# tsinghua-fib-lab/PIML

Hardware: AMD Instinct MI355X
Metric: agent-pair force evals/sec + simulated steps/sec, 4096-agent GC scene (higher is better)
Workload: dtype f32

## Files before the change

include/piml_hip_tuning.h:

```cpp
#ifndef PIML_HIP_TUNING_H
#define PIML_HIP_TUNING_H

#include "piml_hip.h"

#ifdef __cplusplus
extern "C" {
#endif

int piml_timer_create(void** event);
int piml_timer_record(void* event, void* stream);
int piml_timer_elapsed_ms(void* start, void* stop, float* ms);
int piml_timer_destroy(void* event);

int piml_trace_begin(void);
int piml_trace_mark(const char* name, void* stream);
int piml_trace_end(char* names, int names_cap, float* us, int us_cap);

int piml_probe_arith(const float* rx, const float* ry, const float* hx, const float* hy,
                     float* dist, float* cosv, int n, void* stream);

long long piml_encoder_split_tiles(long long tiles);
long long piml_encoder_split_tiles_train(long long tiles);
int piml_encoder_products(int split_bf16);
int piml_rowdecoder_products(int split_bf16);
int piml_encoder_dw2(int layer_split);
int piml_encoder_fused_bwd(int on);
int piml_encoder_sums_bwd(int form);
int piml_encoder_sums_dec_slots(int on);
int piml_encoder_compact_rows(int on);
int piml_relfeat_pack_form(int form);
int piml_relfeat_pack_plan(int form, int waves, int obstacle_workgroups, int nbr, int has_head, int has_fold, int skip_f32,
                           int* pack_blocks, int* share);
int piml_relfeat_pack_tail_blocks(int b, int nb, int total, int* out, int cap);
int piml_relfeat_plan(int C, int N, int M, int focal_count, int topk_ped, int topk_obs, int part, int has_pack, int* waves,
                      int* resident, int* split, int* agent_tiles, int* obstacle_tiles);
int piml_pinnsf_streams_init(void);

#ifdef __cplusplus
}
#endif
#endif
```

piml_amd/_lib.py:

```python
import ctypes
import os

import torch

_HERE = os.path.dirname(os.path.abspath(__file__))
LIB_PATH = os.environ.get('PIML_LIB') or os.path.join(_HERE, 'libpiml_hip.so')
ABI_VERSION = 35
COMPACT_MAX_AGENTS = 16384
COMPACT_SLOTS = 256

_lib = None

_i, _f, _p, _z = ctypes.c_int, ctypes.c_float, ctypes.c_void_p, ctypes.c_size_t
_ll = ctypes.c_longlong
_d = ctypes.c_double


class EncoderBranch(ctypes.Structure):
    _fields_ = [('x', _p), ('rows', _ll), ('in_dim', _i), ('k', _i),
                ('w1', _p), ('b1', _p), ('w2', _p), ('b2', _p), ('w3', _p), ('b3', _p),
                ('scale', _f), ('h1', _p), ('h2', _p), ('msgs', _p), ('g_pooled', _p), ('g_msgs', _p),
                ('g2', _p), ('g1', _p), ('g_x', _p), ('partials', _p), ('grads', _p), ('packed', _p), ('relu_mask', _p),
                ('keep_bits', _p), ('drop_state', _p), ('drop_p', _f), ('sum_a', _p), ('sum_b', _p),
                ('nbr_idx', _p), ('plan', _p)]
# ... 201 lines not shown
    'piml_colsum_blocks': [_z, _i],
    'piml_act_bwd_colsum': [_p, _p, _z, _i, _p, _p, _p, _p],
    'piml_sum_leading': [_p, _i, _z, _p, _p],
    'piml_act_bwd_colsum_stage1': [_p, _p, _z, _i, _p, _p, _p, _p],
    'piml_layer_reduce': [_p, _i, _z, _p, _p, _i, _i, _p, _p],
    'piml_scale_ksum_fwd': [_p, _p, _z, _i, _i, _f, _p, _p, _p, _p],
    'piml_ksum_blocks': [_z, _i],
    'piml_scale_ksum_bwd': [_p, _p, _z, _i, _i, _f, _p, _p, _p, _p],
    'piml_dropout_keep_bits': [_p, _ll, _i, _f, _i, _p, _p],
    'piml_timer_create': [ctypes.POINTER(_p)],
    'piml_timer_record': [_p, _p],
    'piml_timer_elapsed_ms': [_p, _p, ctypes.POINTER(_f)],
    'piml_timer_destroy': [_p],
    'piml_trace_begin': [],
    'piml_trace_mark': [ctypes.c_char_p, _p],
    'piml_trace_end': [ctypes.c_char_p, _i, ctypes.POINTER(_f), _i],
    'piml_probe_arith': [_p, _p, _p, _p, _p, _p, _i, _p],
    'piml_encoder_partial_floats': [],
    'piml_encoder_pack_floats': [],
    'piml_encoder_split_tiles': [_ll],
    'piml_encoder_split_tiles_train': [_ll],
    'piml_multi_copy': [ctypes.POINTER(_p), ctypes.POINTER(_p), ctypes.POINTER(_z), _i, _p],
    'piml_rollout_prologue': [_p] * 8 + [_i] * 4 + [_p] * 11 + [_p],
    'piml_rollout_losses_blocks': [_i, _i],
    'piml_rollout_losses': [_p, _p, _ll, _p, _p, _p, _p, _p, _i, _i, _i, _f, _p, _p, _p, _p, _p, _p, _p],
    'piml_rollout_losses_bwd': [_p, _p, _p, _p, _p, _p, _ll, _p, _p],
    'piml_rollout_losses_frames': [_p, _p, _ll, _p, _p, ctypes.POINTER(_p), _i, _p, _i, _i, _i, _f, _f, _f, _p, _p, _p, _p, _p, _p, _p],
    'piml_rollout_losses_frames_bwd': [_p, _p, _p, _p, _f, _f, _p, _p, _p, _ll, _p, _p],
    'piml_collision_pred_loss_blocks': [_ll, _i],
    'piml_collision_pred_loss': [ctypes.POINTER(_p), ctypes.POINTER(_p), _i, _ll, _i, _i, _p, _i, _i, _f, _p, _p, _p, _p, _p],
    'piml_collision_pred_loss_bwd': [_p, _p, _ll, _p, _p],
    'piml_adam_tickets': [],
    'piml_adam_step': [ctypes.POINTER(_p)] * 5 + [ctypes.POINTER(_ll), _i, ctypes.c_double, ctypes.c_double, ctypes.c_double, ctypes.c_double, ctypes.c_double, _p, _p],
    'piml_pointwise_losses_blocks': [_ll, _ll, _i],
    'piml_pointwise_losses': [_p, _p, _ll, _ll, _p, _ll, _f, _p, _i, _p, _p, _p, _p, _p],
    'piml_p2p_alloc': [_z, ctypes.POINTER(_p)],
    'piml_p2p_free': [_p],
    'piml_p2p_export': [_p, _p],
    'piml_p2p_open': [_p, ctypes.POINTER(_p)],
    'piml_p2p_close': [_p],
    'piml_p2p_copy': [_p, _p, _z, _p],
    'piml_allgather_state_p2p': [_p, _z, _i, _i, ctypes.POINTER(_p), ctypes.POINTER(_p), ctypes.c_uint, ctypes.c_uint, _p, _p],
    'piml_encoder_products': [_i],
    'piml_relfeat_pack_form': [_i],
    'piml_relfeat_pack_plan': [_i, _i, _i, _i, _i, _i, _i, ctypes.POINTER(_i), ctypes.POINTER(_i)],
    'piml_relfeat_pack_tail_blocks': [_i, _i, _i, ctypes.POINTER(_i), _i],
    'piml_relfeat_plan': [_i] * 8 + [ctypes.POINTER(_i)] * 5,
    'piml_rowdecoder_products': [_i],
    'piml_encoder_dw2': [_i],
    'piml_encoder_fused_bwd': [_i],
    'piml_encoder_sums_bwd': [_i],
    'piml_encoder_sums_dec_slots': [_i],
    'piml_encoder_compact_rows': [_i],
    'piml_encoder_pack': [ctypes.POINTER(EncoderBranch), _i, _p],
    'piml_encoder_workgroups': [ctypes.POINTER(EncoderBranch), _i, ctypes.POINTER(_i)],
    'piml_encoder_fwd': [ctypes.POINTER(EncoderBranch), _i, _p],
    'piml_encoder_fwd_packed': [ctypes.POINTER(EncoderBranch), _i, _p],
    'piml_encoder_bwd': [ctypes.POINTER(EncoderBranch), _i, _p],
    'piml_encoder_bwd_acc': [ctypes.POINTER(EncoderBranch), _i, _i, _p],
    'piml_encoder_ksum': [_p, _ll, _i, _p, _p],
    'piml_decoder_pack_floats': [],
    'piml_decoder_partial_floats': [],
    'piml_decoder_workgroups': [_ll],
    'piml_decoder_fwd': [ctypes.POINTER(DecoderBranch), _i, _p, _f, _p, _p],
    'piml_decoder_bwd': [ctypes.POINTER(DecoderBranch), _i, _p, _p, _f, _p, _p],
    'piml_rowdecoder_slots': [_ll],
    'piml_rowdecoder_fwd': [ctypes.POINTER(DecoderBranch), _i, _p],
    'piml_rowdecoder_fwd_packed': [ctypes.POINTER(DecoderBranch), _i, _p],
    'piml_rowdecoder_bwd': [ctypes.POINTER(DecoderBranch), _i, _p],
    'piml_rowdecoder_bwd_acc': [ctypes.POINTER(DecoderBranch), _i, _i, _p],
    'piml_collision_head_pack_floats': [],
    'piml_collision_head_fwd': [_p, _ll, _p, _p, _p, _p, _p, _p, _p],
    'piml_head64_partial_floats': [],
    'piml_head64_slots': [_ll],
    'piml_head64_fwd': [ctypes.POINTER(Head64), _p],
    'piml_head64_bwd': [ctypes.POINTER(Head64), _p],
    'piml_head64_bwd_acc': [ctypes.POINTER(Head64), _i, _p],
    'piml_corrector_partial_floats': [_i],
    'piml_corrector_slots': [_i, _ll, _i],
    'piml_corrector_fwd': [ctypes.POINTER(Corrector), _p],
    'piml_corrector_bwd': [ctypes.POINTER(Corrector), _i, _p],
    'piml_pinnsf_pool_h2_ok': [ctypes.POINTER(EncoderBranch), _i],
    'piml_pinnsf_pool_train_ok': [ctypes.POINTER(EncoderBranch), _i],
    'piml_pinnsf_pool_msgs_ok': [ctypes.POINTER(EncoderBranch), _i],
    'piml_pinnsf_streams_init': [],
    'piml_pinnsf_pack_flush': [],
    'piml_pinnsf_slot_sums_flush': [],
    'piml_pinnsf_pack': [ctypes.POINTER(EncoderBranch), ctypes.POINTER(DecoderBranch), _i, ctypes.POINTER(CollisionHead),
                         _i, _p],
    'piml_pinnsf_fwd': [ctypes.POINTER(EncoderBranch), ctypes.POINTER(DecoderBranch), _i, ctypes.POINTER(CollisionHead),
                        _p, _f, _p, _i, _p],
    'piml_pinnsf_bwd': [ctypes.POINTER(EncoderBranch), ctypes.POINTER(DecoderBranch), _i, _p, _p, _f, _p, _i, _p],
    'piml_comm_available': [],
    'piml_comm_unique_id': [_p],
    'piml_comm_init': [ctypes.POINTER(_p), _i, _i, _p],
    'piml_comm_destroy': [_p],
    'piml_allgather_state': [_p, _p, _z, _p, _p],
    'piml_reducescatter_grad': [_p, _p, _p, _z, _p],
    'piml_allreduce_sum': [_p, _p, _z, _p],
    'piml_relfeat_fwd_self': [_p, _p, _p, _p, _i, _p, _p, _p, _i, _i, _i, _i, _i, _i, _i, _f, _f, _f, _f, _p, _p, _p, _p, _p, _p, _p],
    'piml_relfeat_bwd_self': [_p, _p, _p, _p, _p, _p, _i, _p, _i, _i, _i, _i, _i, _i, _p, _p, _p, _p],
    'piml_relfeat_fwd_tick': [_p, _p, _p, _p, _i, _p, _p, _i, _i, _i, _i, _i, _i, _i, _f, _f, _f, _f,
                              _p, _p, _p, _i, _p, _p, _p, _p],
    'piml_relfeat_self_fwd': [_p, _p, _p, _p, _i, _i, _i, _i, _i, _i, _f, _f, _f, _f, _p, _p, _p, _p, _p, _p, _p],
    'piml_relfeat_self_fwd_part': [_i, _p, _p, _p, _p, _i, _i, _i, _i, _i, _i, _f, _f, _f, _f, _p, _p, _p, _p, _p, _p, _p],
    'piml_relfeat_self_bwd': [_p, _p, _p, _p, _p, _p, _p, _i, _i, _i, _i, _i, _p, _p, _p, _p],
# ... 167 lines not shown
```

piml_amd/csrc/encoder_x3.hip:

```cpp
#include <cstdlib>

#include "common.hpp"
#include "encoder.hpp"
#include "philox.hpp"
#include "x3.hpp"

namespace piml {

struct Pieces {
    u32x4 hi[8], mid[8], lo[8];
};

__device__ __forceinline__ void split_tile(const f32x16 (&in)[4], Pieces& P) {
#pragma unroll
    for (int kb = 0; kb < 8; ++kb) {
        const f32x16& a = in[kb >> 1];
        const int r = 8 * (kb & 1);
        unsigned hi[4], mid[4], lo[4];
#pragma unroll
        for (int d = 0; d < 4; ++d) split3(a[r + 2 * d], a[r + 2 * d + 1], hi[d], mid[d], lo[d]);
        P.hi[kb] = (u32x4){hi[0], hi[1], hi[2], hi[3]};
        P.mid[kb] = (u32x4){mid[0], mid[1], mid[2], mid[3]};
        P.lo[kb] = (u32x4){lo[0], lo[1], lo[2], lo[3]};
    }
// ... 89 lines not shown
}
__device__ __forceinline__ void pool_block_k(const f32x16& ab, int blk, int k, long long tile, long long agents, int lane,
                                             float* __restrict__ part_a, float* __restrict__ part_b) {
    if (k == 6) {
        switch ((int)(tile % 3)) {
            case 0: pool_block<6, 0>(ab, blk, tile, agents, lane, part_a, part_b); break;
            case 1: pool_block<6, 1>(ab, blk, tile, agents, lane, part_a, part_b); break;
            default: pool_block<6, 2>(ab, blk, tile, agents, lane, part_a, part_b); break;
        }
    } else if (k == 10) {
        switch ((int)(tile % 5)) {
            case 0: pool_block<10, 0>(ab, blk, tile, agents, lane, part_a, part_b); break;
            case 1: pool_block<10, 1>(ab, blk, tile, agents, lane, part_a, part_b); break;
            case 2: pool_block<10, 2>(ab, blk, tile, agents, lane, part_a, part_b); break;
            case 3: pool_block<10, 3>(ab, blk, tile, agents, lane, part_a, part_b); break;
            default: pool_block<10, 4>(ab, blk, tile, agents, lane, part_a, part_b); break;
        }
    } else {
        pool_block<2, 0>(ab, blk, tile, agents, lane, part_a, part_b);
    }
}
__device__ __forceinline__ void store_rows_block(const f32x16& ab, int blk, float* __restrict__ out, long long tile, long long R, int lane) {
    const int j = lane & 31, h = lane >> 5;
    float* __restrict__ base = out + (tile * 32 + 4 * h) * EH + 32 * blk + j;
    const long long left = R - tile * 32 - 4 * h;
    if (R - tile * 32 >= 32) {
#pragma unroll
        for (int r = 0; r < 16; ++r) base[((r & 3) + 8 * (r >> 2)) * EH] = ab[r];
    } else {
#pragma unroll
        for (int r = 0; r < 16; ++r)
            if ((r & 3) + 8 * (r >> 2) < left) base[((r & 3) + 8 * (r >> 2)) * EH] = ab[r];
    }
}

__device__ __forceinline__ void pool_rows_k(const f32x16 (&a)[4], int k, long long tile, long long agents, int lane, float* __restrict__ part_a,
                                            float* __restrict__ part_b) {
    if (k == 6) {
        switch ((int)(tile % 3)) {
            case 0: pool_rows<6, 0>(a, tile, agents, lane, part_a, part_b); break;
            case 1: pool_rows<6, 1>(a, tile, agents, lane, part_a, part_b); break;
            default: pool_rows<6, 2>(a, tile, agents, lane, part_a, part_b); break;
        }
    } else if (k == 10) {
        switch ((int)(tile % 5)) {
            case 0: pool_rows<10, 0>(a, tile, agents, lane, part_a, part_b); break;
            case 1: pool_rows<10, 1>(a, tile, agents, lane, part_a, part_b); break;
            case 2: pool_rows<10, 2>(a, tile, agents, lane, part_a, part_b); break;
            case 3: pool_rows<10, 3>(a, tile, agents, lane, part_a, part_b); break;
            default: pool_rows<10, 4>(a, tile, agents, lane, part_a, part_b); break;
        }
    } else {
        pool_rows<2, 0>(a, tile, agents, lane, part_a, part_b);
    }
}

template <int DROP, bool EXCH = false>
__global__ __launch_bounds__(ENC_THREADS) void enc_fwd_x3_kernel(EncArgs A) {
    extern __shared__ __align__(16) float lds[];
    const int tid = threadIdx.x, lane = tid & 63, wave = uniform((int)(threadIdx.x >> 6));
    const int b = (A.nbr > 1 && (int)blockIdx.x >= A.wg_split) ? 1 : 0;
    const piml_encoder_branch J = b ? A.br[1] : A.br[0];
    const int wg0 = b ? A.wg_split : 0;
    const int nwg = b ? (int)gridDim.x - A.wg_split : (A.nbr > 1 ? A.wg_split : (int)gridDim.x);
    const long long R = J.rows;
    const int IN = J.in_dim;
    const long long ntiles = (R + 31) >> 5;
    const long long first = (long long)wave * nwg + ((int)blockIdx.x - wg0);
    const long long stride = (long long)nwg * ENC_WAVES;
    if (A.zero)
        for (int e = blockIdx.x * ENC_THREADS + tid; e < A.zero_n; e += gridDim.x * ENC_THREADS) A.zero[e] = 0.f;
    unsigned long long gseed = 0, goff = 0;
    if (DROP == 2) { gseed = A.gen_state[0]; goff = A.gen_state[1]; }
    if ((long long)((int)blockIdx.x - wg0) >= ntiles) {
        if (DROP == 2 && tid == 0) dropout_advance(A.gen_state, goff, gridDim.x);
        return;
    }

    const float* x3 = J.packed + PACK_F32;
    float xb[4];
    ENC_STAMP(0, false);
    load_x(xb, J.x, first, ntiles, R, IN, lane);
    stage_linear<X3_IMG>(lds, x3, tid);
    stage_linear<1024 + 384>(lds + X3_FWD_F32, J.packed + 32768, tid);
    __syncthreads();
    u32x4 w3r[W3_ROUNDS];
    {
        const u32x4* src = reinterpret_cast<const u32x4*>(x3 + X3_IMG);
#pragma unroll
        for (int r = 0; r < W3_ROUNDS; ++r) {
            const int e = r * ENC_THREADS + tid;
            w3r[r] = src[e < W3_N4 ? e : 0];
        }
    }
    bool w3_pending = true;
    ENC_STAMP(1, false);
    if (EXCH && DROP) {
        land_w3(w3r, lds, tid);
        w3_pending = false;
    }
    ENC_STAMP(2, false);

    for (long long tile = first; tile < ntiles; tile += stride) {
        int lane_t = lane;
        asm volatile("" : "+v"(lane_t));
        const u32x4* W2hm = reinterpret_cast<const u32x4*>(lds) + lane_t;
// ... 174 lines not shown
    ENC_STAMP(7, false);
    ENC_STAMP(8, true);
    if (w3_pending) land_w3(w3r, lds, tid);
    if (DROP == 2 && tid == 0) dropout_advance(A.gen_state, goff, gridDim.x);
}

__device__ __forceinline__ float add_halves(float x) {
    const unsigned u = __float_as_uint(x);
    const auto r = __builtin_amdgcn_permlane32_swap(u, u, false, false);
    return __uint_as_float(r[0]) + __uint_as_float(r[1]);
}

template <int K, int PH>
__device__ __forceinline__ void pool_rows(const f32x16 (&a)[4], long long tile, long long agents, int lane, float* __restrict__ part_a,
                                          float* __restrict__ part_b) {
    constexpr int o = (PH * 32) % K;
    constexpr int S = (o + 31) / K + 1;
    const int i = lane & 31;
    const bool h = lane >= 32;
    const long long a0 = (tile * 32) / K;
    float tot[4][S];
#pragma unroll
    for (int blk = 0; blk < 4; ++blk) {
        float sum[S];
#pragma unroll
        for (int s = 0; s < S; ++s) sum[s] = 0.f;
#pragma unroll
        for (int r = 0; r < 16; ++r) {
            const int m0 = (r & 3) + 8 * (r >> 2), s0 = (o + m0) / K, s1 = (o + m0 + 4) / K;
            if (s0 == s1) sum[s0] += a[blk][r];
            else {
                sum[s0] += h ? 0.f : a[blk][r];
                sum[s1] += h ? a[blk][r] : 0.f;
            }
        }
#pragma unroll
        for (int s = 0; s < S; ++s) tot[blk][s] = add_halves(sum[s]);
    }
    float* __restrict__ pa = part_a + a0 * EH + i;
    float* __restrict__ pb = part_b + a0 * EH + i;
    const int left = (int)(agents - a0 < S ? agents - a0 : S);
    if (!h) {
#pragma unroll
        for (int s = 0; s < S; ++s) {
            if (s < left) {
                float* dst = (s == 0 && o != 0) ? pb : pa;
#pragma unroll
                for (int blk = 0; blk < 4; ++blk) dst[s * EH + 32 * blk] = tot[blk][s];
            }
        }
    }
}

__global__ __launch_bounds__(ENC_THREADS) void enc_fwd_pool_x3_kernel(EncArgs A) {
    extern __shared__ __align__(16) float lds[];
    const int tid = threadIdx.x, lane = tid & 63, wave = uniform((int)(threadIdx.x >> 6));
    const int b = (A.nbr > 1 && (int)blockIdx.x >= A.wg_split) ? 1 : 0;
    const piml_encoder_branch J = b ? A.br[1] : A.br[0];
    const int wg0 = b ? A.wg_split : 0;
    const int nwg = b ? (int)gridDim.x - A.wg_split : (A.nbr > 1 ? A.wg_split : (int)gridDim.x);
    const long long R = J.rows;
    const int IN = J.in_dim;
    const long long ntiles = (R + 31) >> 5;
    const long long first = (long long)wave * nwg + ((int)blockIdx.x - wg0);
    const long long stride = (long long)nwg * ENC_WAVES;
    if (A.zero)
        for (int e = blockIdx.x * ENC_THREADS + tid; e < A.zero_n; e += gridDim.x * ENC_THREADS) A.zero[e] = 0.f;
    if ((long long)((int)blockIdx.x - wg0) >= ntiles) return;
    const float* x3 = J.packed + PACK_F32;
    float xb[4];
    load_x(xb, J.x, first, ntiles, R, IN, lane);
    stage_linear<X3_IMG>(lds, x3, tid);
    stage_linear<1024 + 384>(lds + X3_FWD_F32, J.packed + 32768, tid);
    __syncthreads();
    const int k = J.k;
    const long long agents = R / k;
    for (long long tile = first; tile < ntiles; tile += stride) {
        int lane_t = lane;
        asm volatile("" : "+v"(lane_t));
        const u32x4* W2hm = reinterpret_cast<const u32x4*>(lds) + lane_t;
        const u32x4* W2lo = W2hm + X3_HM / 4;
        const float* W1f = lds + X3_FWD_F32;
        const float* bias = W1f + 1024;
        const int h = lane_t >> 5;
        f32x16 a[4];
        Pieces P;
#pragma unroll
        for (int blk = 0; blk < 4; ++blk) {
#pragma unroll
            for (int q = 0; q < 4; ++q) {
                const float4 bq = *reinterpret_cast<const float4*>(bias + feat0(blk, q, h));
                a[blk][4 * q + 0] = bq.x; a[blk][4 * q + 1] = bq.y; a[blk][4 * q + 2] = bq.z; a[blk][4 * q + 3] = bq.w;
            }
#pragma unroll
            for (int s = 0; s < 4; ++s) a[blk] = mfma32(W1f[(blk * 4 + s) * 64 + lane_t], xb[s], a[blk]);
            const float pre0 = a[blk][0];
#pragma unroll
            for (int r = 0; r < 16; ++r) a[blk][r] = relu1(a[blk][r]);
            if (blk == 0) a[0][0] = __builtin_fmaf(pre0, 0.f, a[0][0]);
        }
        split_tile(a, P);
        load_x(xb, J.x, tile + stride, ntiles, R, IN, lane);
#pragma unroll
        for (int blk = 0; blk < 4; ++blk) {
            f32x16 acc, sm;
            const float bv = bias[128 + 32 * blk + (lane_t & 31)];
#pragma unroll
            for (int r = 0; r < 16; ++r) { sm[r] = 0.f; acc[r] = bv; }
#pragma unroll
            for (int kb = 0; kb < 8; ++kb) {
                const int fb = blk * 8 + kb;
                kblock_x3_t(acc, sm, W2hm[(fb * 2) * 64], W2hm[(fb * 2 + 1) * 64], W2lo[fb * 64], P.hi[kb], P.mid[kb], P.lo[kb]);
            }
#pragma unroll
            for (int r = 0; r < 16; ++r) {
                const float pre = acc[r] + sm[r];
                a[blk][r] = blk == 0 ? __builtin_fmaf(pre, 0.f, relu1(pre)) : relu1(pre);
            }
        }
        pool_rows_k(a, k, tile, agents, lane_t, J.msgs, J.h2);
    }
}


template <bool ROWS>
__device__ __forceinline__ void store_h2_rows(const f32x16 (&a)[4], float* __restrict__ h2, long long tile, long long R, int lane) {
    if (!ROWS) return;
    const int j = lane & 31, h = lane >> 5;
    float* __restrict__ base = h2 + (tile * 32 + 4 * h) * EH + j;
    const long long left = R - tile * 32 - 4 * h;
    if (R - tile * 32 >= 32) {
#pragma unroll
        for (int blk = 0; blk < 4; ++blk)
#pragma unroll
            for (int r = 0; r < 16; ++r) base[((r & 3) + 8 * (r >> 2)) * EH + 32 * blk] = a[blk][r];
    } else {
#pragma unroll
        for (int blk = 0; blk < 4; ++blk)
#pragma unroll
            for (int r = 0; r < 16; ++r)
                if ((r & 3) + 8 * (r >> 2) < left) base[((r & 3) + 8 * (r >> 2)) * EH + 32 * blk] = a[blk][r];
    }
}

constexpr int CP_LDS_CNT = X3_IMG;
constexpr int CP_LDS_LIST = X3_IMG + 1024;
constexpr int CP_ROUNDS0 = 8;
static_assert((CP_LDS_LIST - X3_IMG) * 4 + PIML_COMPACT_MAX_AGENTS * 2 <= (X3_FWD_F32 - X3_IMG) * 4, "the lists fit W3's region");
static_assert(PIML_COMPACT_MAX_AGENTS <= 65536 && PIML_COMPACT_MAX_AGENTS <= 32 * ENC_THREADS, "u16 entries, a 32-bit flag word per thread");

__device__ __forceinline__ bool cp_straddles(int agent, int k) { return ((agent * k) >> 5) != ((agent * k + k - 1) >> 5); }

__device__ __forceinline__ unsigned cp_split_cost(int w0, int tiles0, int tiles1, int nemp) {
    const int w1 = PIML_COMPACT_SLOTS - w0;
    const unsigned c0 = (unsigned)((tiles0 + w0 - 1) / w0) * 6000u;
    const unsigned c1 = (unsigned)((tiles1 + w1 - 1) / w1) * 6000u + (nemp > 0 ? 2500u + 40u * (unsigned)((nemp + w1 - 1) / w1) : 0u);
    return min(c0 > c1 ? c0 : c1, (1u << 23) - 1u);
}

template <int K>
__device__ __forceinline__ void pool_rows_c(const f32x16 (&a)[4], int tile, int nne, const unsigned short* list, int lane,
                                            float* __restrict__ sum_a, float* __restrict__ sum_b) {
    constexpr int S = 32 / K;
    const int i = lane & 31;
    const bool h = lane >= 32;
    float tot[4][S];
#pragma unroll
    for (int blk = 0; blk < 4; ++blk) {
        float sum[S];
#pragma unroll
        for (int s = 0; s < S; ++s) sum[s] = 0.f;
#pragma unroll
        for (int r = 0; r < 16; ++r) {
            const int m0 = (r & 3) + 8 * (r >> 2), s0 = m0 / K, s1 = (m0 + 4) / K;
            if (s0 == s1) {
                if (s0 < S) sum[s0] += a[blk][r];
            } else {
                if (s0 < S) sum[s0] += h ? 0.f : a[blk][r];
                if (s1 < S) sum[s1] += h ? a[blk][r] : 0.f;
            }
        }
#pragma unroll
        for (int s = 0; s < S; ++s) tot[blk][s] = add_halves(sum[s]);
    }
    const int left = nne - S * tile;
    if (!h) {
#pragma unroll
        for (int s = 0; s < S; ++s) {
            if (s < left) {
                const int ag = list[S * tile + s];
                float* __restrict__ dst = sum_a + (size_t)ag * EH + i;
#pragma unroll
                for (int blk = 0; blk < 4; ++blk) dst[32 * blk] = tot[blk][s];
                if (cp_straddles(ag, K)) {
                    float* __restrict__ zb = sum_b + (size_t)ag * EH + i;
#pragma unroll
                    for (int blk = 0; blk < 4; ++blk) zb[32 * blk] = 0.f;
                }
            }
        }
    }
}

template <bool CP>
__device__ __forceinline__ void enc_fwd_sum_body(const EncArgs& A) {
    extern __shared__ __align__(16) float lds[];
    const int tid = threadIdx.x, lane = tid & 63, wave = uniform((int)(threadIdx.x >> 6));
    const int b = (A.nbr > 1 && (int)blockIdx.x >= A.wg_split) ? 1 : 0;
    const piml_encoder_branch J = b ? A.br[1] : A.br[0];
    const int wg0 = b ? A.wg_split : 0;
    const int nwg = b ? (int)gridDim.x - A.wg_split : (A.nbr > 1 ? A.wg_split : (int)gridDim.x);
    const long long R = J.rows;
    const int IN = J.in_dim;
    const bool cp = CP && b == 1;
    long long ntiles = (R + 31) >> 5;
    const long long first = (long long)wave * nwg + ((int)blockIdx.x - wg0);
    const long long stride = (long long)nwg * ENC_WAVES;
    if (A.zero)
        for (int e = blockIdx.x * ENC_THREADS + tid; e < A.zero_n; e += gridDim.x * ENC_THREADS) A.zero[e] = 0.f;
    if (!cp && (long long)((int)blockIdx.x - wg0) >= ntiles) return;
    const float* x3 = J.packed + PACK_F32;
    float xb[4];
    ENC_STAMP(0, false);
    const int k = J.k;
    const int agents = CP ? (int)(R / k) : 0;
    int iv[CP_ROUNDS0];
    if (cp) {
#pragma unroll
        for (int i = 0; i < CP_ROUNDS0; ++i) {
            const int a = i * ENC_THREADS + tid;
            iv[i] = a < agents ? J.nbr_idx[(size_t)a * k] : -1;
        }
    } else {
        load_x(xb, J.x, first, ntiles, R, IN, lane);
    }
    stage_linear<X3_IMG>(lds, x3, tid);
    stage_linear<1024 + 384>(lds + X3_FWD_F32, J.packed + 32768, tid);
    ENC_STAMP(1, true);
    int nne = 0, nemp = 0, S = 1, slot_n = 0, kn = 0;
    bool rowlive = false;
    const unsigned short* list = reinterpret_cast<const unsigned short*>(lds + CP_LDS_LIST);
    if (cp) {
        int* cnt = reinterpret_cast<int*>(lds + CP_LDS_CNT);
        unsigned short* lw = reinterpret_cast<unsigned short*>(lds + CP_LDS_LIST);
        const int rounds = (agents + ENC_THREADS - 1) / ENC_THREADS;
        unsigned flags = 0;
#pragma unroll
        for (int i = 0; i < CP_ROUNDS0; ++i) flags |= (iv[i] >= 0 ? 1u : 0u) << i;
        for (int i = CP_ROUNDS0; i < rounds; ++i) {
            const int a = i * ENC_THREADS + tid;
            const int v = a < agents ? J.nbr_idx[(size_t)a * k] : -1;
            flags |= (v >= 0 ? 1u : 0u) << i;
        }
        for (int i = 0; i < rounds; ++i) {
            const unsigned long long bal = __ballot((flags >> i) & 1u);
            if (lane == 0) cnt[i * ENC_WAVES + wave] = __popcll(bal);
        }
// ... 39 lines not shown
            for (int c = tid; c < nne; c += ENC_THREADS) J.plan[CP_LISTS + c] = list[c];
            for (int e = tid; e < nemp; e += ENC_THREADS) J.plan[CP_LISTS + apad + e] = list[agents - 1 - e];
            __syncthreads();
            if (tid == 0) {
                const int w0 = cnt[257] & 255;
                J.plan[0] = nne; J.plan[1] = nemp; J.plan[2] = (int)ntiles; J.plan[3] = w0; J.plan[4] = PIML_COMPACT_SLOTS - w0;
            }
        }
    } else {
        __syncthreads();
    }
    ENC_STAMP(2, false);
    auto load_xc = [&](long long tile) {
        const int idx = S * (int)tile + slot_n;
        const bool ok = tile < ntiles && rowlive && idx < nne;
        const long long row = ok ? (long long)list[idx] * k + kn : 0;
#pragma unroll
        for (int s = 0; s < 4; ++s) {
            const int c = 2 * s + (lane >> 5);
            xb[s] = (ok && c < IN) ? J.x[row * IN + c] : 0.f;
        }
    };
    if (cp) load_xc(first);
    const long long agents_d = R / k;
    for (long long tile = first; tile < ntiles; tile += stride) {
        int lane_t = lane;
        asm volatile("" : "+v"(lane_t));
        const u32x4* W2hm = reinterpret_cast<const u32x4*>(lds) + lane_t;
        const u32x4* W2lo = W2hm + X3_HM / 4;
        const float* W1f = lds + X3_FWD_F32;
        const float* bias = W1f + 1024;
        const int h = lane_t >> 5;
        f32x16 a[4];
        Pieces P;
#pragma unroll
        for (int blk = 0; blk < 4; ++blk) {
#pragma unroll
            for (int q = 0; q < 4; ++q) {
                const float4 bq = *reinterpret_cast<const float4*>(bias + feat0(blk, q, h));
                a[blk][4 * q + 0] = bq.x; a[blk][4 * q + 1] = bq.y; a[blk][4 * q + 2] = bq.z; a[blk][4 * q + 3] = bq.w;
            }
#pragma unroll
            for (int s = 0; s < 4; ++s) a[blk] = mfma32(W1f[(blk * 4 + s) * 64 + lane_t], xb[s], a[blk]);
#pragma unroll
            for (int r = 0; r < 16; ++r) a[blk][r] = relu1(a[blk][r]);
        }
        uint2* mrow = reinterpret_cast<uint2*>(J.relu_mask) + (tile * 2) * 64 + lane_t;
        mrow[0] = make_uint2(sign_bits(a[0], a[1]), sign_bits(a[2], a[3]));
        ENC_STAMP(3, false);
        split_tile(a, P);
        ENC_STAMP(4, false);
        if (cp) load_xc(tile + stride);
        else load_x(xb, J.x, tile + stride, ntiles, R, IN, lane);
#pragma unroll
        for (int blk = 0; blk < 4; ++blk) {
            f32x16 acc, sm;
            const float bv = bias[128 + 32 * blk + (lane_t & 31)];
#pragma unroll
            for (int r = 0; r < 16; ++r) { sm[r] = 0.f; acc[r] = bv; }
#pragma unroll
            for (int kb = 0; kb < 8; ++kb) {
                const int fb = blk * 8 + kb;
                kblock_x3_t(acc, sm, W2hm[(fb * 2) * 64], W2hm[(fb * 2 + 1) * 64], W2lo[fb * 64], P.hi[kb], P.mid[kb], P.lo[kb]);
            }
#pragma unroll
            for (int r = 0; r < 16; ++r) a[blk][r] = relu1(acc[r] + sm[r]);
        }
        ENC_STAMP(5, false);
        mrow[64] = make_uint2(sign_bits(a[0], a[1]), sign_bits(a[2], a[3]));
        if (J.h2) store_h2_rows<true>(a, J.h2, tile, R, lane_t);
        ENC_STAMP(6, false);
        if (cp) {
            if (k == 10) pool_rows_c<10>(a, (int)tile, nne, list, lane_t, J.sum_a, J.sum_b);
            else if (k == 6) pool_rows_c<6>(a, (int)tile, nne, list, lane_t, J.sum_a, J.sum_b);
            else pool_rows_c<2>(a, (int)tile, nne, list, lane_t, J.sum_a, J.sum_b);
        } else {
            pool_rows_k(a, k, tile, agents_d, lane_t, J.sum_a, J.sum_b);
        }
        ENC_STAMP(7, false);
    }
    if (cp && nemp > 0) {
        const int nwav = nwg * ENC_WAVES, idle = nwav - (int)ntiles;
        const int q = idle > 0 ? (int)first - (int)ntiles : (int)first, share = idle > 0 ? idle : nwav;
        if (q >= 0) {
            const float2 hc = reinterpret_cast<const float2*>(J.packed + PACK_ZROW + EH)[lane];
            const float2 v = make_float2((float)k * hc.x, (float)k * hc.y);
            for (int e = q; e < nemp; e += share) {
                const int ag = list[agents - 1 - e];
                reinterpret_cast<float2*>(J.sum_a + (size_t)ag * EH)[lane] = v;
                if (cp_straddles(ag, k)) reinterpret_cast<float2*>(J.sum_b + (size_t)ag * EH)[lane] = make_float2(0.f, 0.f);
            }
        }
    }
    ENC_STAMP(8, true);
}
__global__ __launch_bounds__(ENC_THREADS) void enc_fwd_sum_x3_kernel(EncArgs A) { enc_fwd_sum_body<false>(A); }
__global__ __launch_bounds__(ENC_THREADS) void enc_fwd_sum_x3_cp_kernel(EncArgs A) { enc_fwd_sum_body<true>(A); }

constexpr int X3_SPLIT_LDS_BYTES = 2 * 2 * 4 * 3 * 2 * 64 * 16;

template <int DROP>
__global__ __launch_bounds__(512) void enc_fwd_split_x3_kernel(EncArgs A, int pairs0) {
    extern __shared__ __align__(16) float lds[];
    u32x4* exch = reinterpret_cast<u32x4*>(lds);
    const int tid = threadIdx.x, lane = tid & 63, wave = __builtin_amdgcn_readfirstlane(tid >> 6);
    const int b = (int)blockIdx.x >= pairs0 ? 1 : 0;
    const piml_encoder_branch J = b ? A.br[1] : A.br[0];
    const int t = wave >> 2, blk = wave & 3;
    const long long R = J.rows;
    const int IN = J.in_dim;
    const long long tile = ((long long)blockIdx.x - (b ? pairs0 : 0)) * 2 + t;
    const int j = lane & 31, h = lane >> 5;
    const long long row = tile * 32 + j;
    const bool valid = row < R;
    if (A.zero)
        for (int e = blockIdx.x * 512 + tid; e < A.zero_n; e += gridDim.x * 512) A.zero[e] = 0.f;
    const unsigned long long goff = DROP == 2 ? A.gen_state[1] : 0ull;
    const u32x4* W2hm = reinterpret_cast<const u32x4*>(J.packed + PACK_F32) + lane;
    const u32x4* W2lo = W2hm + X3_HM / 4;
    const u32x4* W3hm = reinterpret_cast<const u32x4*>(J.packed + PACK_F32 + X3_IMG) + lane;
    const u32x4* W3lo = W3hm + X3_HM / 4;
    const float* W1g = J.packed + 32768;
    const float* bias = J.packed + 32768 + 1024;
    u32x4 wf[8][3];
#pragma unroll
    for (int kb = 0; kb < 8; ++kb) {
        const int fb = blk * 8 + kb;
        wf[kb][0] = W2hm[(fb * 2) * 64]; wf[kb][1] = W2hm[(fb * 2 + 1) * 64]; wf[kb][2] = W2lo[fb * 64];
    }
    float xb[4], w1[4];
#pragma unroll
    for (int s = 0; s < 4; ++s) {
        const int c = 2 * s + h;
        xb[s] = (valid && c < IN) ? J.x[(valid ? row : 0) * IN + c] : 0.f;
        w1[s] = W1g[(blk * 4 + s) * 64 + lane];
    }
    float4 bq[4], bqn[4];
#pragma unroll
    for (int q = 0; q < 4; ++q) bq[q] = *reinterpret_cast<const float4*>(bias + feat0(blk, q, h));
    f32x16 acc, sm;
    auto init = [&]() {
#pragma unroll
        for (int q = 0; q < 4; ++q) { acc[4 * q] = bq[q].x; acc[4 * q + 1] = bq[q].y; acc[4 * q + 2] = bq[q].z; acc[4 * q + 3] = bq[q].w; }
#pragma unroll
        for (int r = 0; r < 16; ++r) sm[r] = 0.f;
    };
    auto store = [&](float* dst, float sc) {
        if (dst && valid) {
            float* o = dst + row * EH;
#pragma unroll
// ... 422 lines not shown
        __syncthreads();
    }
    if (blk == 0 && J.g_x) {
        float gx[8];
#pragma unroll
        for (int c = 0; c < 8; ++c) gx[c] = 0.f;
#pragma unroll
        for (int bp = 0; bp < 4; ++bp)
#pragma unroll
            for (int q = 0; q < 4; ++q) {
                __builtin_amdgcn_sched_barrier(0);
#pragma unroll
                for (int u = 0; u < 4; ++u) {
                    const int f = feat0(bp, q, h) + u;
                    const float4 wa = W1r[2 * f], wb = W1r[2 * f + 1];
                    const float v = g1x[((t * 4 + bp) * 16 + 4 * q + u) * 64 + lane];
                    gx[0] = __fmaf_rn(wa.x, v, gx[0]); gx[1] = __fmaf_rn(wa.y, v, gx[1]);
                    gx[2] = __fmaf_rn(wa.z, v, gx[2]); gx[3] = __fmaf_rn(wa.w, v, gx[3]);
                    gx[4] = __fmaf_rn(wb.x, v, gx[4]); gx[5] = __fmaf_rn(wb.y, v, gx[5]);
                    gx[6] = __fmaf_rn(wb.z, v, gx[6]); gx[7] = __fmaf_rn(wb.w, v, gx[7]);
                }
            }
#pragma unroll
        for (int c = 0; c < 8; ++c) gx[c] += __shfl_xor(gx[c], 32, 64);
        if (valid) {
            float* o = J.g_x + row * IN + 4 * h;
            const int left = IN - 4 * h;
            const float s0 = h ? gx[4] : gx[0], s1 = h ? gx[5] : gx[1], s2 = h ? gx[6] : gx[2], s3 = h ? gx[7] : gx[3];
            if (left > 0) o[0] = s0;
            if (left > 1) o[1] = s1;
            if (left > 2) o[2] = s2;
            if (left > 3) o[3] = s3;
        }
    }
}


int enc_x3_set_attributes() {
    auto set = [](const void* f, int bytes) { return (int)hipFuncSetAttribute(f, hipFuncAttributeMaxDynamicSharedMemorySize, bytes); };
    if (int e = set(reinterpret_cast<const void*>(enc_bwd_dx_split_x3_kernel<false>), X3_DXS_LDS_BYTES)) return e;
    if (int e = set(reinterpret_cast<const void*>(enc_bwd_dx_split_x3_kernel<true>), X3_DXS_LDS_BYTES)) return e;
    if (int e = set(reinterpret_cast<const void*>(enc_fwd_split_x3_kernel<0>), X3_SPLIT_LDS_BYTES)) return e;
    if (int e = set(reinterpret_cast<const void*>(enc_fwd_split_x3_kernel<1>), X3_SPLIT_LDS_BYTES)) return e;
    if (int e = set(reinterpret_cast<const void*>(enc_fwd_split_x3_kernel<2>), X3_SPLIT_LDS_BYTES)) return e;
    const void* dx[4] = {reinterpret_cast<const void*>(enc_bwd_dx_x3_kernel<false, false>),
                         reinterpret_cast<const void*>(enc_bwd_dx_x3_kernel<true, false>),
                         reinterpret_cast<const void*>(enc_bwd_dx_x3_kernel<false, true>),
                         reinterpret_cast<const void*>(enc_bwd_dx_x3_kernel<true, true>)};
    for (const void* f : dx)
        if (int e = set(f, X3_DX_LDS_BYTES)) return e;
    if (int e = set(reinterpret_cast<const void*>(enc_fwd_pool_x3_kernel), X3_FWD_LDS_BYTES)) return e;
    if (int e = set(reinterpret_cast<const void*>(enc_fwd_sum_x3_kernel), X3_FWD_LDS_BYTES)) return e;
    if (int e = set(reinterpret_cast<const void*>(enc_fwd_sum_x3_cp_kernel), X3_FWD_LDS_BYTES)) return e;
    if (int e = set(reinterpret_cast<const void*>(enc_fwd_x3_kernel<2, true>), X3_FWD_LDS_BYTES)) return e;
    if (int e = set(reinterpret_cast<const void*>(enc_fwd_x3_kernel<1, true>), X3_FWD_LDS_BYTES)) return e;
    if (int e = set(reinterpret_cast<const void*>(enc_fwd_x3_kernel<0, true>), X3_FWD_LDS_BYTES)) return e;
    if (int e = set(reinterpret_cast<const void*>(enc_fwd_x3_kernel<2>), X3_FWD_LDS_BYTES)) return e;
    if (int e = set(reinterpret_cast<const void*>(enc_fwd_x3_kernel<1>), X3_FWD_LDS_BYTES)) return e;
    return set(reinterpret_cast<const void*>(enc_fwd_x3_kernel<0>), X3_FWD_LDS_BYTES);
}

void enc_x3_launch_bwd_dx(const EncArgs& A, int total, bool mask, bool drop, hipStream_t s) {
    const dim3 g(total), b(ENC_THREADS);
    if (mask && drop) hipLaunchKernelGGL((enc_bwd_dx_x3_kernel<true, true>), g, b, X3_DX_LDS_BYTES, s, A);
    else if (mask) hipLaunchKernelGGL((enc_bwd_dx_x3_kernel<true, false>), g, b, X3_DX_LDS_BYTES, s, A);
    else if (drop) hipLaunchKernelGGL((enc_bwd_dx_x3_kernel<false, true>), g, b, X3_DX_LDS_BYTES, s, A);
    else hipLaunchKernelGGL((enc_bwd_dx_x3_kernel<false, false>), g, b, X3_DX_LDS_BYTES, s, A);
}

void enc_x3_launch_bwd_dx_split(const EncArgs& A, int pairs0, int pairs1, bool drop, hipStream_t s) {
    const dim3 g((unsigned)(pairs0 + pairs1));
    if (drop) hipLaunchKernelGGL(enc_bwd_dx_split_x3_kernel<true>, g, dim3(512), X3_DXS_LDS_BYTES, s, A, pairs0);
    else hipLaunchKernelGGL(enc_bwd_dx_split_x3_kernel<false>, g, dim3(512), X3_DXS_LDS_BYTES, s, A, pairs0);
}

void enc_x3_launch_fwd_split(const EncArgs& A, int pairs0, int pairs1, bool drop, hipStream_t s) {
    const dim3 g((unsigned)(pairs0 + pairs1));
    if (drop && A.gen_state) hipLaunchKernelGGL(enc_fwd_split_x3_kernel<2>, g, dim3(512), X3_SPLIT_LDS_BYTES, s, A, pairs0);
    else if (drop) hipLaunchKernelGGL(enc_fwd_split_x3_kernel<1>, g, dim3(512), X3_SPLIT_LDS_BYTES, s, A, pairs0);
    else hipLaunchKernelGGL(enc_fwd_split_x3_kernel<0>, g, dim3(512), X3_SPLIT_LDS_BYTES, s, A, pairs0);
}

void enc_x3_launch_fwd_pool(const EncArgs& A, int total, hipStream_t s) {
    hipLaunchKernelGGL(enc_fwd_pool_x3_kernel, dim3(total), dim3(ENC_THREADS), X3_FWD_LDS_BYTES, s, A);
}

void enc_x3_launch_fwd_sum(const EncArgs& A, int total, hipStream_t s) {
    if (A.nbr > 1 && A.br[1].plan) hipLaunchKernelGGL(enc_fwd_sum_x3_cp_kernel, dim3(total), dim3(ENC_THREADS), X3_FWD_LDS_BYTES, s, A);
    else hipLaunchKernelGGL(enc_fwd_sum_x3_kernel, dim3(total), dim3(ENC_THREADS), X3_FWD_LDS_BYTES, s, A);
}

void enc_x3_launch_fwd(const EncArgs& A, int total, bool drop, hipStream_t s, bool exch) {
    const dim3 g(total), b(ENC_THREADS);
    if (exch) {
        if (drop && A.gen_state) hipLaunchKernelGGL((enc_fwd_x3_kernel<2, true>), g, b, X3_FWD_LDS_BYTES, s, A);
        else if (drop) hipLaunchKernelGGL((enc_fwd_x3_kernel<1, true>), g, b, X3_FWD_LDS_BYTES, s, A);
        else hipLaunchKernelGGL((enc_fwd_x3_kernel<0, true>), g, b, X3_FWD_LDS_BYTES, s, A);
        return;
    }
    if (drop && A.gen_state) hipLaunchKernelGGL(enc_fwd_x3_kernel<2>, g, b, X3_FWD_LDS_BYTES, s, A);
    else if (drop) hipLaunchKernelGGL(enc_fwd_x3_kernel<1>, g, b, X3_FWD_LDS_BYTES, s, A);
    else hipLaunchKernelGGL(enc_fwd_x3_kernel<0>, g, b, X3_FWD_LDS_BYTES, s, A);
}

}

#ifdef PIML_ENC_STAMPS
extern "C" __attribute__((visibility("default"))) int piml_enc_stamps(unsigned long long* out) {
    return (int)hipMemcpyFromSymbol(out, HIP_SYMBOL(piml::g_enc_stamps), sizeof(unsigned long long) * 512 * 16);
}
#endif
```

Baseline: 249.9 billion.

## Interleave layer-2 block epilogues with next block's MFMA chain in encoder forward

Adds a software-pipelined layer-2 path in which the pooling and sum epilogue, h2 row stores and relu mask bits of block n are spread across the MFMA slots of block n+1, fenced by scheduling barriers. It also uses buffer-resource stores with out-of-range offsets to mask inactive lanes. Weight loads are double-buffered one step ahead. The aim is to hide epilogue VALU and store latency behind matrix instructions. The cost is higher register pressure and more template instantiations, and the path is on by default with an env switch to turn it off.

```diff
diff --git a/include/piml_hip_tuning.h b/include/piml_hip_tuning.h
--- a/include/piml_hip_tuning.h
+++ b/include/piml_hip_tuning.h
@@ -28,6 +28,7 @@
 int piml_encoder_sums_bwd(int form);
 int piml_encoder_sums_dec_slots(int on);
 int piml_encoder_compact_rows(int on);
+int piml_encoder_fwd_tail(int form);
 int piml_relfeat_pack_form(int form);
 int piml_relfeat_pack_plan(int form, int waves, int obstacle_workgroups, int nbr, int has_head, int has_fold, int skip_f32,
                            int* pack_blocks, int* share);
diff --git a/piml_amd/_lib.py b/piml_amd/_lib.py
--- a/piml_amd/_lib.py
+++ b/piml_amd/_lib.py
@@ -277,6 +277,7 @@
     'piml_encoder_sums_bwd': [_i],
     'piml_encoder_sums_dec_slots': [_i],
     'piml_encoder_compact_rows': [_i],
+    'piml_encoder_fwd_tail': [_i],
     'piml_encoder_pack': [ctypes.POINTER(EncoderBranch), _i, _p],
     'piml_encoder_workgroups': [ctypes.POINTER(EncoderBranch), _i, ctypes.POINTER(_i)],
     'piml_encoder_fwd': [ctypes.POINTER(EncoderBranch), _i, _p],
diff --git a/piml_amd/csrc/encoder_x3.hip b/piml_amd/csrc/encoder_x3.hip
--- a/piml_amd/csrc/encoder_x3.hip
+++ b/piml_amd/csrc/encoder_x3.hip
@@ -165,6 +165,168 @@
         }
     } else {
         pool_rows<2, 0>(a, tile, agents, lane, part_a, part_b);
+    }
+}
+
+#define FT_SLOT(MF, FILL)                        \
+    do {                                         \
+        MF;                                      \
+        __builtin_amdgcn_sched_barrier(0);       \
+        FILL;                                    \
+        __builtin_amdgcn_sched_barrier(0);       \
+    } while (0)
+
+constexpr unsigned FT_OUT = 0x80000000u;
+constexpr int FT_STEPS = 40;
+
+__device__ __forceinline__ bool cp_straddles(int agent, int k);
+__device__ __forceinline__ constexpr int ft_rho(int r) { return (r & 3) + 8 * (r >> 2); }
+__device__ __forceinline__ __amdgpu_buffer_rsrc_t ft_rsrc(const void* base, long long bytes) {
+    return __builtin_amdgcn_make_buffer_rsrc(const_cast<void*>(base), 0, (int)(bytes < 0 ? 0 : bytes), 0x00020000);
+}
+
+struct FwdTailOut {
+    float* h2;
+    unsigned* relu_mask;
+    float *part_a, *part_b;
+    long long rows;
+    long long agents;
+    int nne;
+    const unsigned short* list;
+};
+
+template <bool TRAIN, bool CPT, int K, int PH>
+__device__ __forceinline__ void layer2_block_tails(const Pieces& P, const float* lds, int lane_t, long long tile, const FwdTailOut& T) {
+    constexpr int O = CPT ? 0 : (PH * 32) % K;
+    constexpr int S = CPT ? 32 / K : (O + 31) / K + 1;
+    constexpr bool ROWS = TRAIN && !CPT;
+    static_assert(S <= 16 && 24 + S <= FT_STEPS, "a sum per free slot");
+    const u32x4* W2hm = reinterpret_cast<const u32x4*>(lds) + lane_t;
+    const u32x4* W2lo = W2hm + X3_HM / 4;
+    const float* bias = lds + X3_FWD_F32 + 1024;
+    const int i = lane_t & 31;
+    const bool h = lane_t >= 32;
+
+    const long long rows_left = T.rows - tile * 32;
+    const __amdgpu_buffer_rsrc_t rs_h2 =
+        ft_rsrc(ROWS ? T.h2 + tile * 32 * EH : nullptr, ROWS && T.h2 ? (rows_left < 32 ? rows_left : 32) * (EH * 4) : 0);
+    const unsigned vo_row = (unsigned)((4 * (lane_t >> 5)) * EH + i) * 4u;
+    __amdgpu_buffer_rsrc_t rs_a, rs_b;
+    unsigned vo_a[S], vo_b[S];
+    if (CPT) {
+        rs_a = ft_rsrc(T.part_a, T.agents * (EH * 4));
+        rs_b = ft_rsrc(T.part_b, T.agents * (EH * 4));
+        const int left = T.nne - S * (int)tile;
+#pragma unroll
+        for (int s = 0; s < S; ++s) {
+            const int idx = S * (int)tile + s;
+            const int ag = T.list[idx < T.nne ? idx : 0];
+            const bool on = !h && s < left;
+            vo_a[s] = on ? ((unsigned)ag * EH + i) * 4u : FT_OUT;
+            vo_b[s] = (K != 2 && on && cp_straddles(ag, K)) ? vo_a[s] : FT_OUT;
+        }
+    } else {
+        const long long a0 = (tile * 32) / K;
+        const long long have = T.agents - a0 < S ? T.agents - a0 : S;
+        rs_a = ft_rsrc(T.part_a + a0 * EH, have * (EH * 4));
+        rs_b = ft_rsrc(T.part_b + a0 * EH, have > 0 ? EH * 4 : 0);
+#pragma unroll
+        for (int s = 0; s < S; ++s) vo_a[s] = vo_b[s] = h ? FT_OUT : (unsigned)(s * EH + i) * 4u;
+    }
+    unsigned* mword = T.relu_mask + ((tile * 2 + 1) * 64 + lane_t) * 2;
+
+    u32x4 w[2][3];
+    auto load_w = [&](int fb) {
+        w[fb & 1][0] = W2hm[(fb * 2) * 64];
+        w[fb & 1][1] = W2hm[(fb * 2 + 1) * 64];
+        w[fb & 1][2] = W2lo[fb * 64];
+    };
+    f32x16 prev;
+    float sum[S];
+    unsigned m16 = 0, mlow = 0;
+
+    auto tail = [&](int pb, int f) {
+        if (pb < 0 || f < 0) return;
+        if (f < 16) {
+            if (f == 0) {
+                m16 = 0;
+#pragma unroll
+                for (int s = 0; s < S; ++s) sum[s] = 0.f;
+            }
+            const int m0 = ft_rho(f), s0 = (O + m0) / K, s1 = (O + m0 + 4) / K;
+            if (s0 == s1) {
+                if (s0 < S) sum[s0 < S ? s0 : 0] += prev[f];
+            } else {
+                if (s0 < S) sum[s0 < S ? s0 : 0] += h ? 0.f : prev[f];
+                if (s1 < S) sum[s1 < S ? s1 : 0] += h ? prev[f] : 0.f;
+            }
+            if (TRAIN) asm volatile("v_cmp_gt_f32 vcc, %1, 0\n\tv_addc_co_u32 %0, vcc, %0, %0, vcc" : "+v"(m16) : "v"(prev[15 - f]) : "vcc");
+            return;
+        }
+        if (f < 32) {
+            const int r = f - 16;
+            if (ROWS) __builtin_amdgcn_raw_buffer_store_b32(__float_as_uint(prev[r]), rs_h2, (int)(vo_row + (unsigned)(ft_rho(r) * EH + 32 * pb) * 4u), 0, 0);
+            if (r < S) sum[r < S ? r : 0] = add_halves(sum[r < S ? r : 0]);
+        }
+        if (f >= 24 && f - 24 < S) {
+            const int s = f - 24;
+            const bool to_b = !CPT && s == 0 && O != 0;
+            __builtin_amdgcn_raw_buffer_store_b32(__float_as_uint(sum[s]), to_b ? rs_b : rs_a, (int)(vo_a[s] + 128u * pb), 0, 0);
+            if (CPT && K != 2) __builtin_amdgcn_raw_buffer_store_b32(0u, rs_b, (int)(vo_b[s] + 128u * pb), 0, 0);
+        }
+        if (TRAIN && f == 32) {
+            if (pb & 1) mword[pb >> 1] = mlow | (m16 << 16);
+            else mlow = m16;
+        }
+    };
+
+    load_w(0);
+#pragma unroll
+    for (int blk = 0; blk < 4; ++blk) {
+        f32x16 acc, sm;
+        const float bv = bias[128 + 32 * blk + i];
+#pragma unroll
+        for (int r = 0; r < 16; ++r) { sm[r] = 0.f; acc[r] = bv; }
+#pragma unroll
+        for (int kb = 0; kb < 8; ++kb) {
+            const int fb = blk * 8 + kb;
+            const u32x4 (&o)[3] = w[fb & 1];
+            FT_SLOT(sm = mfma_bf(P.hi[kb], o[2], sm), if (fb + 1 < 32) load_w(fb + 1));
+            FT_SLOT(sm = mfma_bf(P.mid[kb], o[1], sm), tail(blk - 1, kb * 5 + 0));
+            FT_SLOT(sm = mfma_bf(P.lo[kb], o[0], sm), tail(blk - 1, kb * 5 + 1));
+            FT_SLOT(sm = mfma_bf(P.hi[kb], o[1], sm), tail(blk - 1, kb * 5 + 2));
+            FT_SLOT(sm = mfma_bf(P.mid[kb], o[0], sm), tail(blk - 1, kb * 5 + 3));
+            FT_SLOT(acc = mfma_bf(P.hi[kb], o[0], acc), tail(blk - 1, kb * 5 + 4));
+        }
+#pragma unroll
+        for (int r = 0; r < 16; ++r) {
+            const float pre = acc[r] + sm[r];
+            prev[r] = (!TRAIN && blk == 0) ? __builtin_fmaf(pre, 0.f, relu1(pre)) : relu1(pre);
+        }
+    }
+    ENC_STAMP(5, false);
+#pragma unroll
+    for (int f = 0; f < FT_STEPS; ++f) tail(3, f);
+}
+
+template <bool TRAIN>
+__device__ __forceinline__ void layer2_block_tails_k(const Pieces& P, const float* lds, int lane_t, int k, long long tile, const FwdTailOut& T) {
+    if (k == 6) {
+        switch ((int)(tile % 3)) {
+            case 0: layer2_block_tails<TRAIN, false, 6, 0>(P, lds, lane_t, tile, T); break;
+            case 1: layer2_block_tails<TRAIN, false, 6, 1>(P, lds, lane_t, tile, T); break;
+            default: layer2_block_tails<TRAIN, false, 6, 2>(P, lds, lane_t, tile, T); break;
+        }
+    } else if (k == 10) {
+        switch ((int)(tile % 5)) {
+            case 0: layer2_block_tails<TRAIN, false, 10, 0>(P, lds, lane_t, tile, T); break;
+            case 1: layer2_block_tails<TRAIN, false, 10, 1>(P, lds, lane_t, tile, T); break;
+            case 2: layer2_block_tails<TRAIN, false, 10, 2>(P, lds, lane_t, tile, T); break;
+            case 3: layer2_block_tails<TRAIN, false, 10, 3>(P, lds, lane_t, tile, T); break;
+            default: layer2_block_tails<TRAIN, false, 10, 4>(P, lds, lane_t, tile, T); break;
+        }
+    } else {
+        layer2_block_tails<TRAIN, false, 2, 0>(P, lds, lane_t, tile, T);
     }
 }
 
@@ -445,7 +607,8 @@
     }
 }
 
-__global__ __launch_bounds__(ENC_THREADS) void enc_fwd_pool_x3_kernel(EncArgs A) {
+template <bool TAIL>
+__device__ __forceinline__ void enc_fwd_pool_body(const EncArgs& A) {
     extern __shared__ __align__(16) float lds[];
     const int tid = threadIdx.x, lane = tid & 63, wave = uniform((int)(threadIdx.x >> 6));
     const int b = (A.nbr > 1 && (int)blockIdx.x >= A.wg_split) ? 1 : 0;
@@ -494,6 +657,11 @@
         }
         split_tile(a, P);
         load_x(xb, J.x, tile + stride, ntiles, R, IN, lane);
+        if (TAIL) {
+            FwdTailOut T = {nullptr, nullptr, J.msgs, J.h2, R, agents, 0, nullptr};
+            layer2_block_tails_k<false>(P, lds, lane_t, k, tile, T);
+            continue;
+        }
 #pragma unroll
         for (int blk = 0; blk < 4; ++blk) {
             f32x16 acc, sm;
@@ -514,6 +682,8 @@
         pool_rows_k(a, k, tile, agents, lane_t, J.msgs, J.h2);
     }
 }
+__global__ __launch_bounds__(ENC_THREADS) void enc_fwd_pool_x3_kernel(EncArgs A) { enc_fwd_pool_body<false>(A); }
+__global__ __launch_bounds__(ENC_THREADS) void enc_fwd_pool_x3_pb_kernel(EncArgs A) { enc_fwd_pool_body<true>(A); }
 
 
 template <bool ROWS>
@@ -595,7 +765,7 @@
     }
 }
 
-template <bool CP>
+template <bool CP, bool TAIL>
 __device__ __forceinline__ void enc_fwd_sum_body(const EncArgs& A) {
     extern __shared__ __align__(16) float lds[];
     const int tid = threadIdx.x, lane = tid & 63, wave = uniform((int)(threadIdx.x >> 6));
@@ -741,6 +911,19 @@
         ENC_STAMP(4, false);
         if (cp) load_xc(tile + stride);
         else load_x(xb, J.x, tile + stride, ntiles, R, IN, lane);
+        if (TAIL) {
+            FwdTailOut T = {J.h2, reinterpret_cast<unsigned*>(J.relu_mask), J.sum_a, J.sum_b, R, agents_d, nne, list};
+            if (cp) {
+                if (k == 10) layer2_block_tails<true, true, 10, 0>(P, lds, lane_t, tile, T);
+                else if (k == 6) layer2_block_tails<true, true, 6, 0>(P, lds, lane_t, tile, T);
+                else layer2_block_tails<true, true, 2, 0>(P, lds, lane_t, tile, T);
+            } else {
+                layer2_block_tails_k<true>(P, lds, lane_t, k, tile, T);
+            }
+            ENC_STAMP(6, false);
+            ENC_STAMP(7, false);
+            continue;
+        }
 #pragma unroll
         for (int blk = 0; blk < 4; ++blk) {
             f32x16 acc, sm;
@@ -783,8 +966,10 @@
     }
     ENC_STAMP(8, true);
 }
-__global__ __launch_bounds__(ENC_THREADS) void enc_fwd_sum_x3_kernel(EncArgs A) { enc_fwd_sum_body<false>(A); }
-__global__ __launch_bounds__(ENC_THREADS) void enc_fwd_sum_x3_cp_kernel(EncArgs A) { enc_fwd_sum_body<true>(A); }
+__global__ __launch_bounds__(ENC_THREADS) void enc_fwd_sum_x3_kernel(EncArgs A) { enc_fwd_sum_body<false, false>(A); }
+__global__ __launch_bounds__(ENC_THREADS) void enc_fwd_sum_x3_cp_kernel(EncArgs A) { enc_fwd_sum_body<true, false>(A); }
+__global__ __launch_bounds__(ENC_THREADS) void enc_fwd_sum_x3_pb_kernel(EncArgs A) { enc_fwd_sum_body<false, true>(A); }
+__global__ __launch_bounds__(ENC_THREADS) void enc_fwd_sum_x3_cp_pb_kernel(EncArgs A) { enc_fwd_sum_body<true, true>(A); }
 
 constexpr int X3_SPLIT_LDS_BYTES = 2 * 2 * 4 * 3 * 2 * 64 * 16;
 
@@ -1313,6 +1498,9 @@
     if (int e = set(reinterpret_cast<const void*>(enc_fwd_pool_x3_kernel), X3_FWD_LDS_BYTES)) return e;
     if (int e = set(reinterpret_cast<const void*>(enc_fwd_sum_x3_kernel), X3_FWD_LDS_BYTES)) return e;
     if (int e = set(reinterpret_cast<const void*>(enc_fwd_sum_x3_cp_kernel), X3_FWD_LDS_BYTES)) return e;
+    if (int e = set(reinterpret_cast<const void*>(enc_fwd_pool_x3_pb_kernel), X3_FWD_LDS_BYTES)) return e;
+    if (int e = set(reinterpret_cast<const void*>(enc_fwd_sum_x3_pb_kernel), X3_FWD_LDS_BYTES)) return e;
+    if (int e = set(reinterpret_cast<const void*>(enc_fwd_sum_x3_cp_pb_kernel), X3_FWD_LDS_BYTES)) return e;
     if (int e = set(reinterpret_cast<const void*>(enc_fwd_x3_kernel<2, true>), X3_FWD_LDS_BYTES)) return e;
     if (int e = set(reinterpret_cast<const void*>(enc_fwd_x3_kernel<1, true>), X3_FWD_LDS_BYTES)) return e;
     if (int e = set(reinterpret_cast<const void*>(enc_fwd_x3_kernel<0, true>), X3_FWD_LDS_BYTES)) return e;
@@ -1342,13 +1530,25 @@
     else hipLaunchKernelGGL(enc_fwd_split_x3_kernel<0>, g, dim3(512), X3_SPLIT_LDS_BYTES, s, A, pairs0);
 }
 
+static int g_fwd_tail = !(getenv("PIML_ENC_FWD_TAIL") && atoi(getenv("PIML_ENC_FWD_TAIL")) == 0);
+
 void enc_x3_launch_fwd_pool(const EncArgs& A, int total, hipStream_t s) {
-    hipLaunchKernelGGL(enc_fwd_pool_x3_kernel, dim3(total), dim3(ENC_THREADS), X3_FWD_LDS_BYTES, s, A);
+    const dim3 g(total), b(ENC_THREADS);
+    if (g_fwd_tail) hipLaunchKernelGGL(enc_fwd_pool_x3_pb_kernel, g, b, X3_FWD_LDS_BYTES, s, A);
+    else hipLaunchKernelGGL(enc_fwd_pool_x3_kernel, g, b, X3_FWD_LDS_BYTES, s, A);
 }
 
 void enc_x3_launch_fwd_sum(const EncArgs& A, int total, hipStream_t s) {
-    if (A.nbr > 1 && A.br[1].plan) hipLaunchKernelGGL(enc_fwd_sum_x3_cp_kernel, dim3(total), dim3(ENC_THREADS), X3_FWD_LDS_BYTES, s, A);
-    else hipLaunchKernelGGL(enc_fwd_sum_x3_kernel, dim3(total), dim3(ENC_THREADS), X3_FWD_LDS_BYTES, s, A);
+    const dim3 g(total), b(ENC_THREADS);
+    const bool cp = A.nbr > 1 && A.br[1].plan;
+    if (g_fwd_tail) {
+        if (cp) hipLaunchKernelGGL(enc_fwd_sum_x3_cp_pb_kernel, g, b, X3_FWD_LDS_BYTES, s, A);
+        else hipLaunchKernelGGL(enc_fwd_sum_x3_pb_kernel, g, b, X3_FWD_LDS_BYTES, s, A);
+    } else if (cp) {
+        hipLaunchKernelGGL(enc_fwd_sum_x3_cp_kernel, g, b, X3_FWD_LDS_BYTES, s, A);
+    } else {
+        hipLaunchKernelGGL(enc_fwd_sum_x3_kernel, g, b, X3_FWD_LDS_BYTES, s, A);
+    }
 }
 
 void enc_x3_launch_fwd(const EncArgs& A, int total, bool drop, hipStream_t s, bool exch) {
@@ -1366,6 +1566,12 @@
 
 }
 
+PIML_API int piml_encoder_fwd_tail(int form) {
+    const int old = piml::g_fwd_tail;
+    if (form >= 0) piml::g_fwd_tail = form ? 1 : 0;
+    return old;
+}
+
 #ifdef PIML_ENC_STAMPS
 extern "C" __attribute__((visibility("default"))) int piml_enc_stamps(unsigned long long* out) {
     return (int)hipMemcpyFromSymbol(out, HIP_SYMBOL(piml::g_enc_stamps), sizeof(unsigned long long) * 512 * 16);
```

Result: no change. 250.8 billion (median of 4 runs) (+0.4%).
